# BlueSwordM/aom-av1-psy

Measured on AMD Instinct MI355X. Metric: SAD-candidates/s, higher is better.
Workload: dtype u8; 1 GPU; sad16x16_modeA_1080p_8bit; frame=1920x1080, bit_depth=8, block=16x16, mode=A: 1 sad16x16 @mv(0,0) + 1 sad16x16x4d (uniform in [-64,64]^2) per block, ring_frame_pairs_per_gpu=64, partition=uniform tile columns (tile_common.c:76-97), one per GPU; no data-path collective

## Files before the change

aom-av1-psy_amd/csrc/sad_sb.hip:

```cpp
#include <type_traits>

#include "common.h"
#include "variance_device.h"
#undef AOMHIP_FOR_BLOCK_SIZES

namespace aomhip {
namespace sb {

template <bool VAR> struct Ac;
template <> struct Ac<false> { uint32_t a = 0; };
template <> struct Ac<true> { uint32_t a = 0, rr = 0, xr = 0, ssum = 0, ss = 0; };
template <bool VAR> struct Res;
template <> struct Res<false> { uint32_t v; };
template <> struct Res<true> { uint32_t v, sse; };
template <typename T> __device__ __forceinline__ uint32_t dot_dword(uint32_t a, uint32_t b, uint32_t acc) {
  if constexpr (sizeof(T) == 1) return __builtin_amdgcn_udot4(a, b, acc, false);
  else return __builtin_amdgcn_udot2(__builtin_bit_cast(__attribute__((__vector_size__(2 * sizeof(unsigned short)))) unsigned short, a),
                                     __builtin_bit_cast(__attribute__((__vector_size__(2 * sizeof(unsigned short)))) unsigned short, b), acc, false);
}

struct __attribute__((packed, aligned(1))) U128 { uint32_t v[4]; };
struct __attribute__((packed, aligned(1))) U64 { uint32_t v[2]; };
struct __attribute__((packed, aligned(1))) U32 { uint32_t v[1]; };
template <int BYTES> struct UnitLoad;
template <> struct UnitLoad<16> { using type = U128; using aligned_type = uint4; };
template <> struct UnitLoad<8> { using type = U64; using aligned_type = uint2; };
template <> struct UnitLoad<4> { using type = U32; using aligned_type = uint32_t; };

template <typename T> __device__ __forceinline__ uint32_t sad_dword(uint32_t a, uint32_t b, uint32_t acc);
template <> __device__ __forceinline__ uint32_t sad_dword<uint8_t>(uint32_t a, uint32_t b, uint32_t acc) {
  return __builtin_amdgcn_sad_u8(a, b, acc);
}
template <> __device__ __forceinline__ uint32_t sad_dword<uint16_t>(uint32_t a, uint32_t b, uint32_t acc) {
  return __builtin_amdgcn_sad_u16(a, b, acc);
}

template <int TPC> __device__ __forceinline__ uint32_t group_sum(uint32_t v) {
  if constexpr (TPC >= 2) v += __builtin_amdgcn_update_dpp(0u, v, 0xB1, 0xf, 0xf, false);
  if constexpr (TPC >= 4) v += __builtin_amdgcn_update_dpp(0u, v, 0x4E, 0xf, 0xf, false);
  if constexpr (TPC >= 8) v += __builtin_amdgcn_update_dpp(0u, v, 0x141, 0xf, 0xf, false);
  if constexpr (TPC >= 16) v += __builtin_amdgcn_update_dpp(0u, v, 0x140, 0xf, 0xf, false);
  if constexpr (TPC >= 32) v += __shfl_xor(v, 16, 64);
  if constexpr (TPC >= 64) v += __shfl_xor(v, 32, 64);
  return v;
}

template <typename T, int W, int H, bool SKIP, int UPL> struct Geom {
  static constexpr int kRowBytes = W * (int)sizeof(T);
  static constexpr int kUnitBytes = kRowBytes < 16 ? kRowBytes : 16;
  static constexpr int kUnitElems = kUnitBytes / (int)sizeof(T);
  static constexpr int kUnitsPerRow = kRowBytes / kUnitBytes;
  static constexpr int kRows = SKIP ? H / 2 : H;
  static constexpr int kUnits = kUnitsPerRow * kRows;
  static constexpr int kTpcRaw = UPL > 0 ? (kUnits >= UPL ? kUnits / UPL : 1) : (kUnits < 16 ? kUnits : 16);
  static constexpr int kTpc = kTpcRaw > 64 ? 64 : kTpcRaw;
  static constexpr int kUnitsPerLane = kUnits / kTpc;
  static constexpr int kRowStep = SKIP ? 2 : 1;
};

template <int BYTES>
__device__ __forceinline__ typename UnitLoad<BYTES>::type lds_unit(const char *lds, unsigned byte_off) {
  const uint32_t *p = reinterpret_cast<const uint32_t *>(lds) + (byte_off >> 2);
  const unsigned sh = byte_off & 3;
  uint32_t d[BYTES / 4 + 1];
#pragma unroll
  for (int i = 0; i <= BYTES / 4; ++i) d[i] = p[i];
  typename UnitLoad<BYTES>::type out;
#pragma unroll
  for (int i = 0; i < BYTES / 4; ++i) out.v[i] = __builtin_amdgcn_alignbyte(d[i + 1], d[i], sh);
  return out;
}
template <int BYTES>
__device__ __forceinline__ typename UnitLoad<BYTES>::type lds_unit_aligned(const char *lds, unsigned byte_off) {
  using A = typename UnitLoad<BYTES>::aligned_type;
  const A t = *reinterpret_cast<const A *>(lds + byte_off);
  typename UnitLoad<BYTES>::type out;
  memcpy(&out, &t, BYTES);
  return out;
}

struct StripArgs {
  int first_frame, n_frames;
  int sb_w, sb_h, range, cells_per_row, cell_rows;
  int xmin, xmax, ymin, ymax, row_end, border;
  int s_xmax, s_ymax, s_row_end, s_border;
  int cpr, pitch, R;
  int scpr, spitch;
  unsigned magic_cpr, magic_scpr, magic_R;
  int ring_off, src_off[2], gdesc_off[2], cdesc_off[2], misc_off, seg_off;
  int gcap, ccap;
  int shift;
  int dbg;
};

__device__ __forceinline__ int uni(int v) { return __builtin_amdgcn_readfirstlane(v); }

#ifndef AOMHIP_SB_DBG_KNOBS
#define AOMHIP_SB_DBG_KNOBS 0
#endif
#ifdef AOMHIP_SB_PROF
__device__ unsigned long long g_sb_prof[32];
#define SB_T(v) const long long v = (long long)__builtin_readcyclecounter()
#define SB_ACC(i, t1, t0) prof_acc[i] += (unsigned long long)((t1) - (t0))
#define SB_DECL unsigned long long prof_acc[8] = { 0, 0, 0, 0, 0, 0, 0, 0 }, prof_wait = 0
#define SB_WAIT(t1, t0) prof_wait += (unsigned long long)((t1) - (t0))
#define SB_FLUSH if (tid == 0 || tid == kThreads) { for (int i_ = 0; i_ < 8; ++i_) atomicAdd(&g_sb_prof[(tid ? 8 : 0) + i_], prof_acc[i_]); } \
  if (lane == 0) atomicAdd(&g_sb_prof[16 + wave], prof_wait);
#else
#define SB_DECL
#define SB_FLUSH
#define SB_T(v)
#define SB_ACC(i, t1, t0)
#define SB_WAIT(t1, t0)
#endif

constexpr int kMirrorMax = 15;
__host__ __device__ constexpr int mirror_rows(int h) { return h - 1 <= kMirrorMax ? h - 1 : 0; }

template <int EVAL, int UPL_, int LOADERS, int RING_N, int SRC_N, int G_N, int C_N> struct Cfg {
  static constexpr int kThreads = EVAL, kUPL = UPL_, kLoaders = LOADERS, kRingN = RING_N, kSrcN = SRC_N, kGN = G_N, kCN = C_N;
  static constexpr int kLT = 64 * LOADERS / 2;
  static constexpr int kAll = EVAL + 64 * LOADERS;
};
using CfgWide = Cfg<512, 2, 8, 6, 4, 2, 1>;
using CfgDeep = Cfg<768, 1, 4, 9, 6, 4, 2>;
template <typename T, int W, int H, bool SKIP, typename C, bool VAR = false>
__global__ __launch_bounds__(C::kAll) void sad_strip_kernel(PlaneView<T> src, PlaneView<T> ref, StripArgs a,
                                                                  const aomhip_sad_x4d_cand *__restrict__ groups,
                                                                  const int32_t *__restrict__ group_off, int n_groups,
                                                                  int64_t group_frame_stride, uint32_t *__restrict__ out4,
                                                                  const aomhip_sad_cand *__restrict__ cands,
                                                                  const int32_t *__restrict__ cand_off, int n_cands,
                                                                  int64_t cand_frame_stride, uint32_t *__restrict__ out1,
                                                                  uint32_t *__restrict__ out4b = nullptr, uint32_t *__restrict__ out1b = nullptr) {
  static_assert(!VAR || (!SKIP && W * H <= 256), "the variance form: whole blocks of at most 256 pixels (32-bit sums)");
  constexpr int kThreads = C::kThreads, UPL = C::kUPL, kRingN = C::kRingN, kSrcN = C::kSrcN, kGN = C::kGN,
                kCN = C::kCN, kLT = C::kLT;
  using G = Geom<T, W, H, SKIP, UPL>;
  using L = typename UnitLoad<G::kUnitBytes>::type;
  extern __shared__ __attribute__((aligned(16))) char lds[];
  constexpr int kES = (int)sizeof(T);
  constexpr int kEpc = 16 / kES;
  constexpr int kPerWg = kThreads / G::kTpc;
  constexpr int kWaves = kThreads / 64;
  constexpr int kAll = C::kAll;
  constexpr int kGenUnroll = G::kUnitsPerLane <= 4 ? G::kUnitsPerLane : 4;
  constexpr int kMirror = mirror_rows(H);
  const int tid = (int)threadIdx.x;
#if AOMHIP_SB_DBG_KNOBS
  const int dbg = a.dbg;
#else
  constexpr int dbg = 0;
#endif
  const int lane = tid & 63;
  const int wave = uni(tid >> 6);
  const bool is_loader = wave >= kWaves;
  const int grp = uni((tid - kThreads) / kLT);
  const int lt = tid - kThreads - grp * kLT;
  const int lane_in_cand = tid % G::kTpc;
  const int slot = tid / G::kTpc;

  int *misc = reinterpret_cast<int *>(lds + a.misc_off);
  uint8_t *active = reinterpret_cast<uint8_t *>(misc + 72);
  for (int i = tid; i < 72; i += kAll) misc[i] = 0;
  __syncthreads();
  {
    const int n_buckets = a.cells_per_row * a.cell_rows;
    for (int b = tid; b < n_buckets; b += kAll) {
      int n = 0;
      if (groups) n += group_off[b + 1] - group_off[b];
      if (cands) n += cand_off[b + 1] - cand_off[b];
      if (n > 0) {
        const int cx = b % a.cells_per_row;
        atomicOr(reinterpret_cast<unsigned *>(&misc[8 + (cx >> 5)]), 1u << (cx & 31));
      }
    }
    __syncthreads();
    if (tid < 64) {
      int count = 0;
      for (int base = 0; base < a.cells_per_row; base += 64) {
        const int cx = base + tid;
        const bool f = cx < a.cells_per_row && ((misc[8 + (cx >> 5)] >> (cx & 31)) & 1);
        const unsigned long long m = __ballot(f);
        if (f) active[count + __popcll(m & ((1ull << tid) - 1))] = (uint8_t)cx;
        count += __popcll(m);
      }
      if (tid == 0) misc[0] = count;
    }
    __syncthreads();
  }
  const int n_active = uni(misc[0]);
  if (n_active == 0) return;
  const int src_off0 = a.src_off[0], src_off1 = a.src_off[1], gdesc_off0 = a.gdesc_off[0], gdesc_off1 = a.gdesc_off[1];
  const int cdesc_off0 = a.cdesc_off[0], cdesc_off1 = a.cdesc_off[1];
  auto src_off_of = [&](int buf) { return buf ? src_off1 : src_off0; };
  auto gdesc_off_of = [&](int buf) { return buf ? gdesc_off1 : gdesc_off0; };
  auto cdesc_off_of = [&](int buf) { return buf ? cdesc_off1 : cdesc_off0; };

  auto run = [&](auto role) {
    constexpr bool kLoader = decltype(role)::value;
    constexpr bool kTab = G::kUnitsPerLane <= 4;
    constexpr int kTabN = kTab ? G::kUnitsPerLane : 1;
    int unit_row_t[kTabN], unit_colb_t[kTabN];
    unsigned unit_roff_t[kTabN], unit_soff_t[kTabN];
    if constexpr (kTab) {
  #pragma unroll
      for (int k = 0; k < G::kUnitsPerLane; ++k) {
        const int u = lane_in_cand + k * G::kTpc;
        unit_row_t[k] = (u / G::kUnitsPerRow) * G::kRowStep;
        unit_colb_t[k] = (u % G::kUnitsPerRow) * G::kUnitBytes;
        unit_roff_t[k] = (unsigned)(unit_row_t[k] * a.pitch + unit_colb_t[k]);
        unit_soff_t[k] = (unsigned)(unit_row_t[k] * a.spitch + unit_colb_t[k]);
      }
    }
    auto unit_row = [&](int k) -> int {
      if constexpr (kTab) return unit_row_t[k]; else return ((lane_in_cand + k * G::kTpc) / G::kUnitsPerRow) * G::kRowStep;
    };
    auto unit_colb = [&](int k) -> int {
      if constexpr (kTab) return unit_colb_t[k]; else return ((lane_in_cand + k * G::kTpc) % G::kUnitsPerRow) * G::kUnitBytes;
    };
    auto unit_roff = [&](int k) -> unsigned {
      if constexpr (kTab) return unit_roff_t[k]; else return (unsigned)(unit_row(k) * a.pitch + unit_colb(k));
    };
    auto unit_soff = [&](int k) -> unsigned {
      if constexpr (kTab) return unit_soff_t[k]; else return (unsigned)(unit_row(k) * a.spitch + unit_colb(k));
    };

    const bool affine = a.n_frames >= 8;
    const int xcd = affine ? (int)(blockIdx.x & 7) : 0;
    const int wg_j = affine ? (int)(blockIdx.x >> 3) : (int)blockIdx.x;
    const int wg_n = affine ? (int)(gridDim.x >> 3) : (int)gridDim.x;
    const int frames_here = affine ? (a.n_frames - xcd + 7) >> 3 : a.n_frames;
    const int n_items = frames_here * n_active;

    SB_DECL;
    for (int item = wg_j; item < n_items; item += wg_n) {
      const int fi = item / n_active;
      const int f_rel = affine ? xcd + 8 * fi : fi;
      const int cx = uni((int)active[item - fi * n_active]);
      const int cell_x0 = cx * a.sb_w;
      const int wx0 = max(((cell_x0 - a.range + a.border) & ~(kEpc - 1)) - a.border, a.xmin);
      const int colmax = min(a.cpr - 1, (a.row_end - wx0) / kEpc - 1);
      const int wx1 = min(wx0 + (colmax + 1) * kEpc, a.xmax);
      const int sx0 = ((cell_x0 + a.s_border) & ~(kEpc - 1)) - a.s_border;
      const int scolmax = min(a.scpr - 1, (a.s_row_end - sx0) / kEpc - 1);
      const int sx1 = min(sx0 + (scolmax + 1) * kEpc, a.s_xmax);
      const char *ref_frame = reinterpret_cast<const char *>(ref.origin + (int64_t)(a.first_frame + f_rel) * ref.frame_stride);
      const char *src_frame = reinterpret_cast<const char *>(src.origin + (int64_t)(a.first_frame + f_rel) * src.frame_stride);
      const int gpitch = ref.stride * kES, sgpitch = src.stride * kES;
      const aomhip_sad_x4d_cand *glist = groups ? groups + (int64_t)f_rel * group_frame_stride : nullptr;
      const aomhip_sad_cand *clist = cands ? cands + (int64_t)f_rel * cand_frame_stride : nullptr;

      struct Batch { int ya, yb, sy0, ns, g0, ng, c0, nc, buf; unsigned first; };
      typedef uint32_t V4 __attribute__((ext_vector_type(4)));
      struct Stage { V4 ring[kRingN]; V4 srcv[kSrcN]; uint32_t g[kGN]; uint32_t c[kCN]; };
      const uint32_t *gwords = groups ? reinterpret_cast<const uint32_t *>(glist) : reinterpret_cast<const uint32_t *>(ref_frame);
      const uint32_t *cwords = cands ? reinterpret_cast<const uint32_t *>(clist) : reinterpret_cast<const uint32_t *>(ref_frame);
      const int gwords_n = groups ? n_groups * 5 : 1, cwords_n = cands ? n_cands * 2 : 1;
      auto request_gen = [&](const Batch &b, Stage &st, int me, int n) {
        const int total_r = (b.yb - b.ya) * a.cpr, total_s = b.ns * a.scpr;
        const char *rb = ref_frame + (int64_t)b.ya * gpitch + (int64_t)wx0 * kES;
        const char *sb_ = src_frame + (int64_t)b.sy0 * sgpitch + (int64_t)sx0 * kES;
  #pragma unroll
        for (int i = 0; i < kRingN; ++i) {
          const unsigned q = (unsigned)max(min(me + i * n, total_r - 1), 0);
          const unsigned row = __umulhi(q, a.magic_cpr), col = q - row * (unsigned)a.cpr;
          st.ring[i] = *reinterpret_cast<const V4 *>(rb + (row * (unsigned)gpitch + (unsigned)min((int)col, colmax) * 16u));
        }
  #pragma unroll
        for (int i = 0; i < kSrcN; ++i) {
          const unsigned q = (unsigned)max(min(me + i * n, total_s - 1), 0);
          const unsigned row = __umulhi(q, a.magic_scpr), col = q - row * (unsigned)a.scpr;
          st.srcv[i] = *reinterpret_cast<const V4 *>(sb_ + (row * (unsigned)sgpitch + (unsigned)min((int)col, scolmax) * 16u));
        }
  #pragma unroll
        for (int i = 0; i < kGN; ++i) st.g[i] = gwords[(unsigned)max(min(b.g0 * 5 + min(me + i * n, b.ng * 5 - 1), gwords_n - 1), 0)];
  #pragma unroll
        for (int i = 0; i < kCN; ++i) st.c[i] = cwords[(unsigned)max(min(b.c0 * 2 + min(me + i * n, b.nc * 2 - 1), cwords_n - 1), 0)];
      };
      auto commit_gen = [&](const Batch &b, const Stage &st, int me, int n) {
        const int total_r = (b.yb - b.ya) * a.cpr, total_s = b.ns * a.scpr;
        const unsigned s_first = (unsigned)((b.ya - a.ymin) % a.R);
  #pragma unroll
        for (int i = 0; i < kRingN; ++i) {
          const unsigned q = (unsigned)(me + i * n);
          if ((int)q < total_r) {
            const unsigned row = __umulhi(q, a.magic_cpr), col = q - row * (unsigned)a.cpr;
            unsigned sl = s_first + row;
            sl = min(sl, sl - (unsigned)a.R);
            const V4 v = st.ring[i];
            *reinterpret_cast<V4 *>(lds + a.ring_off + sl * a.pitch + col * 16) = v;
            if (kMirror > 0 && sl < (unsigned)kMirror)
              *reinterpret_cast<V4 *>(lds + a.ring_off + (sl + a.R) * a.pitch + col * 16) = v;
          }
        }
  #pragma unroll
        for (int i = 0; i < kSrcN; ++i) {
          const unsigned q = (unsigned)(me + i * n);
          if ((int)q < total_s) {
            const unsigned row = __umulhi(q, a.magic_scpr), col = q - row * (unsigned)a.scpr;
            *reinterpret_cast<V4 *>(lds + src_off_of(b.buf) + row * a.spitch + col * 16) = st.srcv[i];
          }
        }
  #pragma unroll
        for (int i = 0; i < kGN; ++i)
          if (me + i * n < b.ng * 5) *reinterpret_cast<uint32_t *>(lds + gdesc_off_of(b.buf) + (me + i * n) * 4) = st.g[i];
  #pragma unroll
        for (int i = 0; i < kCN; ++i)
          if (me + i * n < b.nc * 2) *reinterpret_cast<uint32_t *>(lds + cdesc_off_of(b.buf) + (me + i * n) * 4) = st.c[i];
      };
      auto win_y0 = [&](int cy) { return max(cy * a.sb_h - a.range, a.ymin); };
      auto win_y1 = [&](int cy) { return min(cy * a.sb_h + a.sb_h + a.range, a.ymax); };
      struct Seg { int g0, g1, c0, c1; };
      const int4 *segs = reinterpret_cast<const int4 *>(lds + a.seg_off);
      int4 *wins = reinterpret_cast<int4 *>(lds + a.seg_off) + a.cell_rows, *bats = wins + a.cell_rows;
      auto seg_of = [&](int cy) {
        const int4 v = segs[cy];
        Seg s;
        s.g0 = uni(v.x); s.g1 = uni(v.y); s.c0 = uni(v.z); s.c1 = uni(v.w);
        return s;
      };
      struct Win { int wy0, s0; unsigned wh_ok, sy0, sh_ok; };
      const unsigned ww_ok = (unsigned)(wx1 - wx0 - W), sw_ok = (unsigned)(sx1 - sx0 - W);
      const bool strip_ok = wx1 - wx0 >= W && sx1 - sx0 >= W;
      auto global_unit = [&](const char *frame, int pitch_b, int x, int y, int k) {
        return *reinterpret_cast<const L *>(frame + (int64_t)(y + unit_row(k)) * pitch_b + (int64_t)x * kES + unit_colb(k));
      };
      using AcT = Ac<VAR>;
      using ResT = Res<VAR>;
      auto add_ref = [&](uint32_t sd, uint32_t rd, AcT &acc) {
        if constexpr (VAR) {
          acc.a = sad_dword<T>(rd, 0u, acc.a);
          acc.rr = dot_dword<T>(rd, rd, acc.rr);
          acc.xr = dot_dword<T>(sd, rd, acc.xr);
        } else {
          acc.a = sad_dword<T>(sd, rd, acc.a);
        }
      };
      auto add_src = [&](uint32_t sd, uint32_t &ssum, uint32_t &ss) {
        ssum = sad_dword<T>(sd, 0u, ssum);
        ss = dot_dword<T>(sd, sd, ss);
      };
      auto sad_unit = [&](const L &s, const L &r, AcT acc) {
  #pragma unroll
        for (int i = 0; i < G::kUnitBytes / 4; ++i) {
          add_ref(s.v[i], r.v[i], acc);
          if constexpr (VAR) add_src(s.v[i], acc.ssum, acc.ss);
        }
        return acc;
      };
      auto reduce = [&](const AcT &acc) {
        ResT r;
        if constexpr (VAR) {
          const uint32_t dsum = group_sum<G::kTpc>(acc.ssum - acc.a);
          const uint32_t q = group_sum<G::kTpc>(acc.ss + acc.rr - 2u * acc.xr);
          finish<(sizeof(T) > 1), ilog2v(W * H)>((int64_t)(int32_t)dsum, (uint64_t)q, 8 + a.shift, &r.v, &r.sse);
        } else {
          r.v = ((SKIP ? 2u * group_sum<G::kTpc>(acc.a) : group_sum<G::kTpc>(acc.a)) >> a.shift);
        }
        return r;
      };
// ... 213 lines not shown
                  const L sv = lds_unit_aligned<G::kUnitBytes>(sbuf, soff + unit_soff(k));
                  if constexpr (kKeepSrc) gsrc[k] = sv;
  #pragma unroll
                  for (int j = 0; j < 4; ++j) acc[j] = sad_unit(sv, ring_unit(base[j], slot0[j], k), acc[j]);
                }
              } else {
  #pragma unroll kGenUnroll
                for (int k = 0; k < G::kUnitsPerLane; ++k) {
                  const L sv = lds_unit<G::kUnitBytes>(sbuf, soff + unit_soff(k));
                  if constexpr (kKeepSrc) gsrc[k] = sv;
  #pragma unroll
                  for (int j = 0; j < 4; ++j) acc[j] = sad_unit(sv, ring_unit(base[j], slot0[j], k), acc[j]);
                }
              }
              gsrc_ok = kKeepSrc;
            } else {
  #pragma unroll 1
              for (int j = 0; j < 4; ++j) {
                int jrx = rx[j], jry = ry[j];
                if constexpr (kCoop) {
                  jrx = (int)quad_bcast((unsigned)rx[0], j);
                  jry = (int)quad_bcast((unsigned)ry[0], j);
                }
                const AcT v = generic_ref(gsx, gsy, jrx, jry);
#pragma unroll
                for (int q = 0; q < 4; ++q) {
                  acc[q].a = j == q ? v.a : acc[q].a;
                  if constexpr (VAR) {
                    acc[q].rr = j == q ? v.rr : acc[q].rr; acc[q].xr = j == q ? v.xr : acc[q].xr;
                    acc[q].ssum = j == q ? v.ssum : acc[q].ssum; acc[q].ss = j == q ? v.ss : acc[q].ss;
                  }
                }
              }
            }
            const ResT r0 = reduce(acc[0]), r1 = reduce(acc[1]), r2 = reduce(acc[2]), r3 = reduce(acc[3]);
            if (lane_in_cand == 0) store_group((int64_t)f_rel * n_groups + g0 + i, r0, r1, r2, r3);
          }
          if (has_c) {
            const uint32_t d0 = cd[i * 2], d1 = cd[i * 2 + 1];
            const int sx = (int16_t)d0, sy = (int16_t)(d0 >> 16), rx = (int16_t)d1, ry = (int16_t)(d1 >> 16);
            AcT acc;
            unsigned soff, base;
            int slot0;
            bool in = src_pos(w, sx, sy, soff);
            in = ring_pos(w, rx, ry, base, slot0) && in;
            if (in) {
              const bool reuse = gsrc_ok && sx == gsx && sy == gsy;
              if (__all(reuse)) {
                if constexpr (kKeepSrc) {
  #pragma unroll
                  for (int k = 0; k < G::kUnitsPerLane; ++k) acc = sad_unit(gsrc[k], ring_unit(base, slot0, k), acc);
                }
              } else {
  #pragma unroll kGenUnroll
                for (int k = 0; k < G::kUnitsPerLane; ++k)
                  acc = sad_unit(lds_unit<G::kUnitBytes>(sbuf, soff + unit_soff(k)), ring_unit(base, slot0, k), acc);
              }
            } else {
              acc = generic_ref(sx, sy, rx, ry);
            }
            const ResT rc = reduce(acc);
            if (lane_in_cand == 0) store_cand((int64_t)f_rel * n_cands + c0 + i, rc);
          }
        }
      };

      auto batch_of = [&](int cy) {
        const bool real = cy < a.cell_rows;
        const int cyc = real ? cy : a.cell_rows - 1;
        const Seg sg = seg_of(cyc);
        const int4 bv = bats[cyc];
        Batch b;
        b.ya = uni(bv.x);
        b.yb = real ? b.ya + uni(bv.y) : b.ya;
        b.sy0 = cyc * a.sb_h; b.ns = real ? uni(bv.z) : 0;
        b.first = (unsigned)uni(bv.w);
        b.g0 = sg.g0; b.ng = real ? min(sg.g1 - sg.g0, a.gcap) : 0;
        b.c0 = sg.c0; b.nc = real ? min(sg.c1 - sg.c0, a.ccap) : 0;
        b.buf = cy & 1;
        if ((dbg & 2) && cy > 0) { b.yb = b.ya; b.ns = 0; }
        if (dbg & 8192) { b.ng = 0; b.nc = 0; }
        return b;
      };
      int crowded = 0;
      for (int cy = tid; cy < a.cell_rows; cy += kAll) {
        const int b = cy * a.cells_per_row + cx;
        const int4 sg = make_int4(groups ? group_off[b] : 0, groups ? group_off[b + 1] : 0, cands ? cand_off[b] : 0, cands ? cand_off[b + 1] : 0);
        reinterpret_cast<int4 *>(lds + a.seg_off)[cy] = sg;
        crowded |= (sg.y - sg.x > a.gcap) | (sg.w - sg.z > a.ccap);
        const int wy0 = win_y0(cy), wy1 = win_y1(cy);
        const int sh = min(cy * a.sb_h + a.sb_h, a.s_ymax) - cy * a.sb_h;
        const bool ok = strip_ok && wy1 - wy0 >= H && sh >= H;
        const unsigned wh_ok = strip_ok && wy1 - wy0 >= H ? (unsigned)(wy1 - wy0 - H) : 0u;
        wins[cy] = make_int4(wy0, (wy0 - a.ymin) % a.R, (int)wh_ok, (int)(((unsigned)(sh - H) & 0x7fffffffu) | (ok ? 0x80000000u : 0u)));
        const int ya = cy > 0 ? win_y1(cy - 1) : win_y0(0);
        bats[cy] = make_int4(ya, wy1 - ya, sh, ((ya - a.ymin) % a.R) * a.pitch);
      }
      if (lane == 0) misc[16 + wave] = __ballot(crowded != 0) != 0 ? 1 : 0;
      __syncthreads();
      bool any_crowded;
      {
        const int4 *f = reinterpret_cast<const int4 *>(misc + 16);
        const int4 f0 = f[0], f1 = f[1], f2 = f[2], f3 = f[3];
        any_crowded = uni((f0.x | f0.y | f0.z | f0.w | f1.x | f1.y | f1.z | f1.w | f2.x | f2.y | f2.z | f2.w | f3.x | f3.y | f3.z | f3.w)) != 0;
      }
      SB_T(p0);
      {
        Stage st0;
        const int rows_per_pass = (kRingN * kAll) / a.cpr;
        const Batch b = batch_of(0);
        for (int ya = win_y0(0); ya < win_y1(0); ya += rows_per_pass) {
          Batch p = b;
          p.ya = ya; p.yb = min(ya + rows_per_pass, win_y1(0));
          if (ya != win_y0(0)) { p.ns = 0; p.ng = 0; p.nc = 0; }
          int me = tid;
          asm volatile("" : "+v"(me));
          request_gen(p, st0, me, kAll);
          commit_gen(p, st0, me, kAll);
        }
      }
      unsigned r_goff[kRingN], r_loff[kRingN], s_goff[kSrcN], s_loff[kSrcN];
      int lt_s = lt;
      asm volatile("" : "+v"(lt_s));
#pragma unroll
      for (int i = 0; i < kRingN; ++i) {
        const unsigned q = (unsigned)(lt_s + i * kLT), row = __umulhi(q, a.magic_cpr), col = q - row * (unsigned)a.cpr;
        r_goff[i] = row * (unsigned)gpitch + (unsigned)min((int)col, colmax) * 16u;
        r_loff[i] = row * (unsigned)a.pitch + col * 16u;
      }
  #pragma unroll
      for (int i = 0; i < kSrcN; ++i) {
        const unsigned q = (unsigned)(lt_s + i * kLT), row = __umulhi(q, a.magic_scpr), col = q - row * (unsigned)a.scpr;
        s_goff[i] = row * (unsigned)sgpitch + (unsigned)min((int)col, scolmax) * 16u;
        s_loff[i] = row * (unsigned)a.spitch + col * 16u;
      }
      const unsigned ring_bytes = (unsigned)(a.R * a.pitch);
      auto request = [&](const Batch &b, Stage &st) {
        const char *rb = ref_frame + (int64_t)min(b.ya, a.ymax - 1) * gpitch + (int64_t)wx0 * kES;
        const char *sb_ = src_frame + (int64_t)min(b.sy0, a.s_ymax - 1) * sgpitch + (int64_t)sx0 * kES;
        const unsigned rlim = (unsigned)((b.yb - b.ya) * gpitch), slim = (unsigned)(b.ns * sgpitch);
  #pragma unroll
        for (int i = 0; i < kRingN; ++i) st.ring[i] = *reinterpret_cast<const V4 *>(rb + (r_goff[i] < rlim ? r_goff[i] : 0u));
  #pragma unroll
        for (int i = 0; i < kSrcN; ++i) st.srcv[i] = *reinterpret_cast<const V4 *>(sb_ + (s_goff[i] < slim ? s_goff[i] : 0u));
  #pragma unroll
        for (int i = 0; i < kGN; ++i) st.g[i] = gwords[(unsigned)max(min(b.g0 * 5 + min(lt + i * kLT, b.ng * 5 - 1), gwords_n - 1), 0)];
  #pragma unroll
        for (int i = 0; i < kCN; ++i) st.c[i] = cwords[(unsigned)max(min(b.c0 * 2 + min(lt + i * kLT, b.nc * 2 - 1), cwords_n - 1), 0)];
      };
      auto commit = [&](const Batch &b, const Stage &st) {
        const unsigned rlim = (unsigned)((b.yb - b.ya) * gpitch), slim = (unsigned)(b.ns * sgpitch);
        const unsigned first = b.first;
        const bool mirrored = kMirror > 0 && (first < (unsigned)(kMirror * a.pitch) || first + (unsigned)(b.yb - b.ya) * (unsigned)a.pitch > ring_bytes);
        if (mirrored) {
  #pragma unroll
          for (int i = 0; i < kRingN; ++i)
            if (r_goff[i] < rlim) {
              unsigned t = first + r_loff[i];
              t = min(t, t - ring_bytes);
              const V4 v = st.ring[i];
              *reinterpret_cast<V4 *>(lds + a.ring_off + t) = v;
              if (t < (unsigned)(kMirror * a.pitch)) *reinterpret_cast<V4 *>(lds + a.ring_off + t + ring_bytes) = v;
            }
        } else {
  #pragma unroll
          for (int i = 0; i < kRingN; ++i)
            if (r_goff[i] < rlim) *reinterpret_cast<V4 *>(lds + a.ring_off + first + r_loff[i]) = st.ring[i];
        }
  #pragma unroll
        for (int i = 0; i < kSrcN; ++i)
          if (s_goff[i] < slim)
            *reinterpret_cast<V4 *>(lds + src_off_of(b.buf) + s_loff[i]) = st.srcv[i];
  #pragma unroll
        for (int i = 0; i < kGN; ++i)
          if (lt + i * kLT < b.ng * 5) *reinterpret_cast<uint32_t *>(lds + gdesc_off_of(b.buf) + (lt + i * kLT) * 4) = st.g[i];
  #pragma unroll
        for (int i = 0; i < kCN; ++i)
          if (lt + i * kLT < b.nc * 2) *reinterpret_cast<uint32_t *>(lds + cdesc_off_of(b.buf) + (lt + i * kLT) * 4) = st.c[i];
      };
      const int steps = (dbg & 256) ? 0 : (a.cell_rows + 1) & ~1;
      if constexpr (kLoader) {
        Stage st;
        auto overflow = [&](int cy, bool mine) {
          if (cy >= a.cell_rows) return;
          const Seg cur = seg_of(cy);
          int g = cur.g0 + min(cur.g1 - cur.g0, a.gcap), c = cur.c0 + min(cur.c1 - cur.c0, a.ccap);
          while (g < cur.g1 || c < cur.c1) {
            Batch o;
            o.ya = o.yb = win_y0(0); o.sy0 = 0; o.ns = 0; o.buf = cy & 1;
            o.g0 = g; o.ng = min(cur.g1 - g, a.gcap); o.c0 = c; o.nc = min(cur.c1 - c, a.ccap);
            __syncthreads();
            if (mine) {
              int me = lt;
              asm volatile("" : "+v"(me));
              Stage so;
              request_gen(o, so, me, kLT);
              commit_gen(o, so, me, kLT);
            }
            __syncthreads();
            g += o.ng; c += o.nc;
          }
        };
        Batch held = batch_of(0);
        auto active = [&](int cy) {
          if (dbg & 64) { __syncthreads(); return; }
          SB_T(l0);
          const Batch bc = held;
          SB_T(l1);
#ifdef AOMHIP_SB_PROF
          asm volatile("s_waitcnt vmcnt(0)" ::: "memory");
          SB_T(l1w);
          SB_ACC(7, l1w, l1);
#endif
          commit(bc, st);
          SB_T(l2);
          if (any_crowded) overflow(cy, true);
          SB_T(l3);
          __syncthreads();
          SB_T(l5);
          SB_ACC(0, l1, l0); SB_ACC(1, l2, l1); SB_ACC(2, l3, l2); SB_ACC(4, l5, l3); SB_ACC(5, 1, 0); SB_WAIT(l5, l3);
        };
        auto passive = [&](int cy) {
          if (dbg & 64) { __syncthreads(); return; }
          SB_T(q0);
          held = batch_of(cy + 2);
          request(held, st);
          SB_T(q1);
          if (any_crowded) overflow(cy, false);
          __syncthreads();
          SB_T(q2);
          SB_ACC(3, q1, q0); SB_ACC(6, q2, q1); SB_WAIT(q2, q1);
        };
        if (grp == 0) {
          held = batch_of(1);
          request(held, st);
          __syncthreads();
          for (int cy = 0; cy < steps; cy += 2) {
            active(cy);
            passive(cy + 1);
          }
        } else {
          __syncthreads();
          for (int cy = 0; cy < steps; cy += 2) {
            passive(cy);
            active(cy + 1);
          }
        }
      } else {
        __syncthreads();
        SB_T(p1);
        SB_ACC(5, p1, p0); SB_ACC(6, 1, 0);
        for (int cy = 0; cy < steps; ++cy) {
          if (cy >= a.cell_rows) {
            __syncthreads();
            break;
          }
          if (dbg & (64 | 2048)) { __syncthreads(); continue; }
          const int buf = cy & 1;
          SB_T(t1);
          const Seg cur = seg_of(cy);
          const int4 wv = wins[cy];
          Win w;
          w.wy0 = uni(wv.x);
          w.s0 = uni(wv.y);
          w.wh_ok = (unsigned)uni(wv.z);
          w.sy0 = (unsigned)(cy * a.sb_h);
          w.sh_ok = (unsigned)uni(wv.w) & 0x7fffffffu;
          const bool step_ok = (unsigned)uni(wv.w) >> 31;
          int g = cur.g0, c = cur.c0;
          bool first = true;
          SB_T(t1b);
          SB_ACC(0, t1b, t1);
          do {
            const int ng = min(cur.g1 - g, a.gcap), nc = min(cur.c1 - c, a.ccap);
            if (!first) {
              __syncthreads();
              __syncthreads();
            }
            if (!(dbg & 1)) {
              if (step_ok) {
                eval(w, buf, g, ng, c, nc);
              } else {
                for (int gi = slot; gi < ng; gi += kPerWg) {
                  const uint32_t *e = reinterpret_cast<const uint32_t *>(glist + g + gi);
                  const uint32_t e0 = e[0], e1 = e[1], e2 = e[2], e3 = e[3], e4 = e[4];
                  const int sx = (int16_t)e0, sy = (int16_t)(e0 >> 16);
                  const ResT r0 = reduce(generic_ref(sx, sy, (int16_t)e1, (int16_t)e3));
                  const ResT r1 = reduce(generic_ref(sx, sy, (int16_t)(e1 >> 16), (int16_t)(e3 >> 16)));
                  const ResT r2 = reduce(generic_ref(sx, sy, (int16_t)e2, (int16_t)e4));
                  const ResT r3 = reduce(generic_ref(sx, sy, (int16_t)(e2 >> 16), (int16_t)(e4 >> 16)));
                  if (lane_in_cand == 0) store_group((int64_t)f_rel * n_groups + g + gi, r0, r1, r2, r3);
                }
                for (int ci = slot; ci < nc; ci += kPerWg) {
                  const uint32_t *e = reinterpret_cast<const uint32_t *>(clist + c + ci);
                  const uint32_t e0 = e[0], e1 = e[1];
                  const ResT v = reduce(generic_ref((int16_t)e0, (int16_t)(e0 >> 16), (int16_t)e1, (int16_t)(e1 >> 16)));
                  if (lane_in_cand == 0) store_cand((int64_t)f_rel * n_cands + c + ci, v);
                }
              }
            }
            g += ng; c += nc;
            first = false;
          } while (g < cur.g1 || c < cur.c1);
          SB_T(t2);
          __syncthreads();
          SB_T(t4);
          SB_ACC(1, t2, t1); SB_ACC(3, t4, t2); SB_ACC(4, 1, 0); SB_WAIT(t4, t2);
        }
      }
    }
    SB_FLUSH;
  };
  if (wave >= kWaves / 2 && wave < kWaves) __builtin_amdgcn_s_setprio(1);
  if (is_loader) run(std::true_type{}); else run(std::false_type{});
}

struct SbLaunch {
  hipStream_t stream;
  int grid, threads, upl;
  bool deep;
  size_t lds_bytes;
  StripArgs a;
  const aomhip_sad_x4d_cand *groups;
  const int32_t *group_off;
  int n_groups;
  int64_t gfs;
  uint32_t *out4;
  const aomhip_sad_cand *cands;
  const int32_t *cand_off;
  int n_cands;
  int64_t cfs;
  uint32_t *out1;
  uint32_t *out4b, *out1b;
  bool var;
};

template <typename T, int W, int H, bool SKIP, typename C, bool VAR = false>
static int launch_nt(const SbLaunch &l, const PlaneView<T> &s, const PlaneView<T> &r) {
  auto k = sad_strip_kernel<T, W, H, SKIP, C, VAR>;
  static thread_local size_t granted = 0;
  if (l.lds_bytes > granted) {
    AOMHIP_TRY(hipFuncSetAttribute(reinterpret_cast<const void *>(k), hipFuncAttributeMaxDynamicSharedMemorySize,
                                   (int)l.lds_bytes));
    granted = l.lds_bytes;
  }
  hipLaunchKernelGGL(k, dim3((unsigned)l.grid), dim3(C::kAll), l.lds_bytes, l.stream, s, r, l.a,
                     l.groups, l.group_off, l.n_groups, l.gfs, l.out4, l.cands, l.cand_off, l.n_cands, l.cfs, l.out1, l.out4b, l.out1b);
  AOMHIP_LAUNCH_CHECK();
  return AOMHIP_OK;
}

constexpr bool deep_size(int es, int w, int h) { return es == 1 && w == 16 && h == 16; }
inline bool use_deep(int es, int w, int h, bool skip) {
  if (!deep_size(es, w, h) || skip) return false;
  const char *e = getenv("AOMHIP_SB_CFG");
  return e && e[0] == 'd';
}
template <typename T, int W, int H, bool SKIP>
static int launch(const SbLaunch &l, const PlaneView<T> &s, const PlaneView<T> &r) {
  if constexpr (deep_size((int)sizeof(T), W, H) && !SKIP) {
    if (l.deep) return launch_nt<T, W, H, SKIP, CfgDeep>(l, s, r);
  }
  return launch_nt<T, W, H, SKIP, CfgWide>(l, s, r);
}

#ifdef AOMHIP_SB_ONLY_16
#define AOMHIP_FOR_BLOCK_SIZES(X) X(16, 16)
#else
#define AOMHIP_FOR_BLOCK_SIZES(X)                                                                                \
  X(4, 4) X(4, 8) X(8, 4) X(8, 8) X(8, 16) X(16, 8) X(16, 16) X(16, 32) X(32, 16) X(32, 32) X(32, 64) X(64, 32) \
  X(64, 64) X(64, 128) X(128, 64) X(128, 128) X(4, 16) X(16, 4) X(8, 32) X(32, 8) X(16, 64) X(64, 16)
#endif

#ifdef AOMHIP_SB_ONLY_16
#define AOMHIP_FOR_VAR_BLOCK_SIZES(X) X(16, 16)
#else
#define AOMHIP_FOR_VAR_BLOCK_SIZES(X) X(4, 4) X(4, 8) X(8, 4) X(8, 8) X(8, 16) X(16, 8) X(16, 16) X(4, 16) X(16, 4) X(8, 32) X(32, 8)
#endif

template <typename T>
static int dispatch(const SbLaunch &l, bool skip, const PlaneView<T> &s, const PlaneView<T> &r, int bw, int bh) {
  if (l.var) {
#define X(W, H) \
  if (bw == W && bh == H) return launch_nt<T, W, H, false, CfgWide, true>(l, s, r);
    AOMHIP_FOR_VAR_BLOCK_SIZES(X)
#undef X
    set_error("aomhip_variance_sb_batch: blocks of at most 256 pixels (%dx%d): use aomhip_variance_batch", bw, bh);
    return AOMHIP_ERR_INVALID;
  }
#define X(W, H) \
  if (bw == W && bh == H) return skip ? launch<T, W, H, (H >= 2)>(l, s, r) : launch<T, W, H, false>(l, s, r);
  AOMHIP_FOR_BLOCK_SIZES(X)
#undef X
  set_error("unsupported block size %dx%d", bw, bh);
  return AOMHIP_ERR_INVALID;
}

static unsigned magic_of(int d) { return (unsigned)((0x100000000ull + (unsigned)d - 1) / (unsigned)d); }

}
}

using namespace aomhip;

#ifdef AOMHIP_SB_PROF
extern "C" int aomhip_debug_sb_prof(unsigned long long out[32], int reset) {
  if (hipMemcpyFromSymbol(out, HIP_SYMBOL(sb::g_sb_prof), 256) != hipSuccess) return AOMHIP_ERR_HIP;
  if (reset) { unsigned long long z[32] = {0}; if (hipMemcpyToSymbol(HIP_SYMBOL(sb::g_sb_prof), z, 256) != hipSuccess) return AOMHIP_ERR_HIP; }
  return AOMHIP_OK;
}
#endif

static int sb_batch(aomhip_ctx *ctx, const aomhip_planes *src, const aomhip_planes *ref, int first_frame,
                    int n_frames, int bw, int bh, int flags, int sb_w, int sb_h, int range,
                    int n_buckets, const aomhip_sad_x4d_cand *d_groups,
                    const int32_t *d_group_bucket_offsets, int n_groups, int64_t group_frame_stride,
                    uint32_t *d_out_groups, const aomhip_sad_cand *d_cands,
                    const int32_t *d_cand_bucket_offsets, int n_cands, int64_t cand_frame_stride,
                    uint32_t *d_out_cands, bool var, uint32_t *d_out_groups_b, uint32_t *d_out_cands_b) {
  if (!ctx || !src || !ref || !src->base || !ref->base) {
    set_error("null argument");
    return AOMHIP_ERR_INVALID;
  }
  if ((d_groups && (!d_group_bucket_offsets || !d_out_groups || (var && !d_out_groups_b))) ||
      (d_cands && (!d_cand_bucket_offsets || !d_out_cands || (var && !d_out_cands_b))) || (!d_groups && !d_cands) || (var && flags != 0)) {
    set_error("a list needs its bucket offsets and its output array; at least one list is required");
    return AOMHIP_ERR_INVALID;
  }
  if (!valid_block(bw, bh)) {
    set_error("unsupported block size %dx%d", bw, bh);
    return AOMHIP_ERR_INVALID;
  }
  if (src->bit_depth != ref->bit_depth && !(src->bit_depth > 8 && ref->bit_depth > 8)) {
    set_error("src/ref element types differ");
    return AOMHIP_ERR_INVALID;
  }
  if (n_groups < 0 || n_cands < 0 || n_frames < 0 || first_frame < 0 || first_frame + n_frames > src->n_frames ||
      first_frame + n_frames > ref->n_frames) {
    set_error("frame range out of bounds");
    return AOMHIP_ERR_INVALID;
  }
  if (sb_w < 1 || sb_h < 1 || range < 0 || n_buckets < 0) {
    set_error("bad bucket geometry");
    return AOMHIP_ERR_INVALID;
  }
  const int cells_per_row = (src->width + sb_w - 1) / sb_w;
  const int cell_rows = (src->height + sb_h - 1) / sb_h;
  if (n_buckets != cells_per_row * cell_rows) {
    set_error("n_buckets %d != %d x %d cells of %dx%d over a %dx%d plane", n_buckets, cells_per_row, cell_rows, sb_w, sb_h,
              src->width, src->height);
    return AOMHIP_ERR_INVALID;
  }
  if (cells_per_row > 256) {
    set_error("at most 256 cells per row (%d of width %d)", cells_per_row, sb_w);
    return AOMHIP_ERR_INVALID;
  }
  if (n_buckets == 0 || n_frames == 0) return AOMHIP_OK;
  const int es = ref->bit_depth > 8 ? 2 : 1, epc = 16 / es;
  sb::SbLaunch l;
  sb::StripArgs &a = l.a;
  memset(&a, 0, sizeof(a));
  const bool aligned = (sb_w % epc) == 0 && (range % epc) == 0 && (ref->border % epc) == 0;
  a.cpr = ((sb_w + 2 * range) * es + 15) / 16 + (aligned ? 0 : 1);
  a.pitch = (a.cpr | 1) * 16;
  a.R = 2 * sb_h + 2 * range;
  a.scpr = (sb_w * es + 15) / 16 + (((sb_w % epc) == 0 && (src->border % epc) == 0) ? 0 : 1);
  a.spitch = ((a.scpr & 3) == 0 ? a.scpr + 1 : a.scpr) * 16;
  l.deep = sb::use_deep(es, bw, bh, (flags & AOMHIP_SAD_SKIP_ROWS) != 0);
  const int ring_chunks = l.deep ? sb::CfgDeep::kRingN * sb::CfgDeep::kLT : sb::CfgWide::kRingN * sb::CfgWide::kLT;
  const int src_chunks = l.deep ? sb::CfgDeep::kSrcN * sb::CfgDeep::kLT : sb::CfgWide::kSrcN * sb::CfgWide::kLT;
  const int g_words = l.deep ? sb::CfgDeep::kGN * sb::CfgDeep::kLT : sb::CfgWide::kGN * sb::CfgWide::kLT;
  const int c_words = l.deep ? sb::CfgDeep::kCN * sb::CfgDeep::kLT : sb::CfgWide::kCN * sb::CfgWide::kLT;
  if (sb_h * a.cpr > ring_chunks || sb_h * a.scpr > src_chunks) {
    set_error("a step of %d rows x (%d + %d) bytes exceeds what the loader wavefronts keep in flight (%d + %d KB): use a lower cell",
              sb_h, a.cpr * 16, a.scpr * 16, ring_chunks / 64, src_chunks / 64);
    return AOMHIP_ERR_INVALID;
  }
  const size_t ring_bytes = (size_t)(a.R + sb::mirror_rows(bh)) * a.pitch, cell_bytes = (size_t)sb_h * a.spitch;
  const size_t kLds = 160 * 1024, misc_bytes = 72 * 4 + 256 + (size_t)cell_rows * 48 + 16;
  if (ring_bytes + 2 * cell_bytes + misc_bytes + 4 * 256 > kLds) {
    set_error("LDS ring of %d rows x %d bytes + two %d x %d source cells (%zu bytes) exceed the 160 KB LDS of a CU: "
              "use a lower cell (sb_h) or a narrower one", a.R, a.pitch, sb_w, sb_h, ring_bytes + 2 * cell_bytes);
    return AOMHIP_ERR_INVALID;
  }
  {
    size_t per_buf = (kLds - ring_bytes - 2 * cell_bytes - misc_bytes) / 2;
    if (per_buf > 16 * 1024) per_buf = 16 * 1024;
    int cap = (int)((per_buf - 32) / 28);
    if (cap > g_words / 5) cap = g_words / 5;
    if (cap > c_words / 2) cap = c_words / 2;
    if (const char *e = getenv("AOMHIP_SB_DESC_CAP")) cap = atoi(e) < cap && atoi(e) > 0 ? atoi(e) : cap;
    a.gcap = a.ccap = cap;
    size_t off = 0;
    a.ring_off = 0; off += ring_bytes;
    for (int i = 0; i < 2; ++i) { a.src_off[i] = (int)off; off += cell_bytes; }
    for (int i = 0; i < 2; ++i) {
      a.gdesc_off[i] = (int)off; off += ((size_t)cap * 20 + 15) & ~(size_t)15;
      a.cdesc_off[i] = (int)off; off += ((size_t)cap * 8 + 15) & ~(size_t)15;
    }
    a.misc_off = (int)off; a.seg_off = (int)((off + 72 * 4 + 256 + 15) & ~(size_t)15); off += misc_bytes;
    l.lds_bytes = (off + 15) & ~(size_t)15;
  }
  a.magic_cpr = sb::magic_of(a.cpr); a.magic_scpr = sb::magic_of(a.scpr); a.magic_R = sb::magic_of(a.R);
  a.first_frame = first_frame; a.n_frames = n_frames;
  a.sb_w = sb_w; a.sb_h = sb_h; a.range = range; a.cells_per_row = cells_per_row; a.cell_rows = cell_rows;
  a.xmin = -ref->border; a.xmax = ref->width + ref->border; a.ymin = -ref->border; a.ymax = ref->height + ref->border;
  a.row_end = ref->stride - ref->border; a.border = ref->border;
  a.s_xmax = src->width + src->border; a.s_ymax = src->height + src->border; a.s_row_end = src->stride - src->border;
  a.s_border = src->border;
  a.shift = src->bit_depth == 10 ? 2 : src->bit_depth == 12 ? 4 : 0;
  if (const char *e = getenv("AOMHIP_SB_DBG")) a.dbg = atoi(e);
  l.stream = ctx->stream;
  {
    static thread_local int cus = 0;
    if (!cus) {
      hipDeviceProp_t prop;
      AOMHIP_TRY(hipGetDeviceProperties(&prop, ctx->device));
      cus = prop.multiProcessorCount > 0 ? prop.multiProcessorCount : 256;
    }
    const int per_cu = (int)(kLds / l.lds_bytes) < 1 ? 1 : (int)(kLds / l.lds_bytes);
    l.threads = per_cu >= 2 ? 512 : 1024;
    int grid = cus * (per_cu > 2 ? 2 : per_cu);
    if (const char *e = getenv("AOMHIP_SB_THREADS")) l.threads = atoi(e);
    if (const char *e = getenv("AOMHIP_SB_GRID")) grid = atoi(e);
    grid &= ~7;
    if (grid < 8) grid = 8;
    const int items = n_frames * cells_per_row;
    if (n_frames < 8 && grid > items) grid = items;
    l.grid = grid;
  }
  l.groups = n_groups > 0 ? d_groups : nullptr; l.group_off = d_group_bucket_offsets; l.n_groups = n_groups; l.gfs = group_frame_stride;
  l.out4 = d_out_groups;
  l.cands = n_cands > 0 ? d_cands : nullptr; l.cand_off = d_cand_bucket_offsets; l.n_cands = n_cands; l.cfs = cand_frame_stride;
  l.out1 = d_out_cands;
  l.var = var; l.out4b = d_out_groups_b; l.out1b = d_out_cands_b;
  const bool skip = (flags & AOMHIP_SAD_SKIP_ROWS) != 0;
  if (src->bit_depth == 8) return sb::dispatch<uint8_t>(l, skip, view_of<uint8_t>(*src), view_of<uint8_t>(*ref), bw, bh);
  return sb::dispatch<uint16_t>(l, skip, view_of<uint16_t>(*src), view_of<uint16_t>(*ref), bw, bh);
}

extern "C" int aomhip_sad_sb_batch(aomhip_ctx *ctx, const aomhip_planes *src, const aomhip_planes *ref, int first_frame,
                                   int n_frames, int bw, int bh, int flags, int sb_w, int sb_h, int range,
                                   int n_buckets, const aomhip_sad_x4d_cand *d_groups,
                                   const int32_t *d_group_bucket_offsets, int n_groups, int64_t group_frame_stride,
                                   uint32_t *d_out_groups, const aomhip_sad_cand *d_cands,
                                   const int32_t *d_cand_bucket_offsets, int n_cands, int64_t cand_frame_stride,
                                   uint32_t *d_out_cands) {
  return sb_batch(ctx, src, ref, first_frame, n_frames, bw, bh, flags, sb_w, sb_h, range, n_buckets, d_groups, d_group_bucket_offsets, n_groups,
                  group_frame_stride, d_out_groups, d_cands, d_cand_bucket_offsets, n_cands, cand_frame_stride, d_out_cands, false, nullptr, nullptr);
}

extern "C" int aomhip_variance_sb_batch(aomhip_ctx *ctx, const aomhip_planes *src, const aomhip_planes *ref, int first_frame, int n_frames, int bw,
                                        int bh, int sb_w, int sb_h, int range, int n_buckets, const aomhip_sad_x4d_cand *d_groups,
                                        const int32_t *d_group_bucket_offsets, int n_groups, int64_t group_frame_stride, uint32_t *d_var_groups,
                                        uint32_t *d_sse_groups, const aomhip_sad_cand *d_cands, const int32_t *d_cand_bucket_offsets, int n_cands,
                                        int64_t cand_frame_stride, uint32_t *d_var_cands, uint32_t *d_sse_cands) {
  return sb_batch(ctx, src, ref, first_frame, n_frames, bw, bh, 0, sb_w, sb_h, range, n_buckets, d_groups, d_group_bucket_offsets, n_groups,
                  group_frame_stride, d_var_groups, d_cands, d_cand_bucket_offsets, n_cands, cand_frame_stride, d_var_cands, true, d_sse_groups,
                  d_sse_cands);
}
```

Before: 33.62 billion candidates/s.

## Cache bucket offsets in LDS and overlap prologue loads with setup

The kernel now copies the group and candidate bucket offsets into LDS during the initial scan, when the extra LDS fits without lowering occupancy, so later per-row segment lookups read LDS instead of global memory. The first window prefetch for cell row 0 is issued earlier, before the segment table and loader offset computations, so its global latency overlaps that setup. The prologue also drops an extra __syncthreads that came after the first batch request. Profiling hooks are extended with prologue timers. The costs are more LDS use and a reordered prologue whose synchronisation must stay correct.

```diff
diff --git a/aom-av1-psy_amd/csrc/sad_sb.hip b/aom-av1-psy_amd/csrc/sad_sb.hip
--- a/aom-av1-psy_amd/csrc/sad_sb.hip
+++ b/aom-av1-psy_amd/csrc/sad_sb.hip
@@ -88,6 +88,7 @@
   int scpr, spitch;
   unsigned magic_cpr, magic_scpr, magic_R;
   int ring_off, src_off[2], gdesc_off[2], cdesc_off[2], misc_off, seg_off;
+  int boff_off;
   int gcap, ccap;
   int shift;
   int dbg;
@@ -99,12 +100,15 @@
 #define AOMHIP_SB_DBG_KNOBS 0
 #endif
 #ifdef AOMHIP_SB_PROF
-__device__ unsigned long long g_sb_prof[32];
+__device__ unsigned long long g_sb_prof[40];
 #define SB_T(v) const long long v = (long long)__builtin_readcyclecounter()
 #define SB_ACC(i, t1, t0) prof_acc[i] += (unsigned long long)((t1) - (t0))
-#define SB_DECL unsigned long long prof_acc[8] = { 0, 0, 0, 0, 0, 0, 0, 0 }, prof_wait = 0
+#define SB_DECL unsigned long long prof_acc[8] = { 0, 0, 0, 0, 0, 0, 0, 0 }, prof_pro[8] = { 0, 0, 0, 0, 0, 0, 0, 0 }, prof_wait = 0
+#define SB_PRO(i, t1, t0) prof_pro[i] += (unsigned long long)((t1) - (t0))
+#define SB_DRAIN asm volatile("s_waitcnt vmcnt(0)" ::: "memory")
 #define SB_WAIT(t1, t0) prof_wait += (unsigned long long)((t1) - (t0))
-#define SB_FLUSH if (tid == 0 || tid == kThreads) { for (int i_ = 0; i_ < 8; ++i_) atomicAdd(&g_sb_prof[(tid ? 8 : 0) + i_], prof_acc[i_]); } \
+#define SB_FLUSH if (tid == 0 || tid == kThreads) { for (int i_ = 0; i_ < 8; ++i_) atomicAdd(&g_sb_prof[(tid ? 8 : 0) + i_], prof_acc[i_]); \
+    for (int i_ = (tid ? 6 : 0); i_ < (tid ? 8 : 6); ++i_) atomicAdd(&g_sb_prof[32 + i_], prof_pro[i_]); } \
   if (lane == 0) atomicAdd(&g_sb_prof[16 + wave], prof_wait);
 #else
 #define SB_DECL
@@ -112,6 +116,8 @@
 #define SB_T(v)
 #define SB_ACC(i, t1, t0)
 #define SB_WAIT(t1, t0)
+#define SB_PRO(i, t1, t0)
+#define SB_DRAIN
 #endif
 
 constexpr int kMirrorMax = 15;
@@ -162,14 +168,20 @@
 
   int *misc = reinterpret_cast<int *>(lds + a.misc_off);
   uint8_t *active = reinterpret_cast<uint8_t *>(misc + 72);
+  SB_T(sc0);
   for (int i = tid; i < 72; i += kAll) misc[i] = 0;
   __syncthreads();
   {
     const int n_buckets = a.cells_per_row * a.cell_rows;
+    int *boff = reinterpret_cast<int *>(lds + max(a.boff_off, 0));
     for (int b = tid; b < n_buckets; b += kAll) {
-      int n = 0;
-      if (groups) n += group_off[b + 1] - group_off[b];
-      if (cands) n += cand_off[b + 1] - cand_off[b];
+      const int g0 = groups ? group_off[b] : 0, g1 = groups ? group_off[b + 1] : 0;
+      const int c0 = cands ? cand_off[b] : 0, c1 = cands ? cand_off[b + 1] : 0;
+      if (a.boff_off >= 0) {
+        boff[b] = g0; boff[n_buckets + 1 + b] = c0;
+        if (b == n_buckets - 1) { boff[b + 1] = g1; boff[n_buckets + 2 + b] = c1; }
+      }
+      const int n = (g1 - g0) + (c1 - c0);
       if (n > 0) {
         const int cx = b % a.cells_per_row;
         atomicOr(reinterpret_cast<unsigned *>(&misc[8 + (cx >> 5)]), 1u << (cx & 31));
@@ -190,6 +202,7 @@
     __syncthreads();
   }
   const int n_active = uni(misc[0]);
+  SB_T(sc1);
   if (n_active == 0) return;
   const int src_off0 = a.src_off[0], src_off1 = a.src_off[1], gdesc_off0 = a.gdesc_off[0], gdesc_off1 = a.gdesc_off[1];
   const int cdesc_off0 = a.cdesc_off[0], cdesc_off1 = a.cdesc_off[1];
@@ -234,6 +247,7 @@
     const int n_items = frames_here * n_active;
 
     SB_DECL;
+    SB_PRO(0, sc1, sc0);
     for (int item = wg_j; item < n_items; item += wg_n) {
       const int fi = item / n_active;
       const int f_rel = affine ? xcd + 8 * fi : fi;
@@ -257,7 +271,7 @@
       const uint32_t *gwords = groups ? reinterpret_cast<const uint32_t *>(glist) : reinterpret_cast<const uint32_t *>(ref_frame);
       const uint32_t *cwords = cands ? reinterpret_cast<const uint32_t *>(clist) : reinterpret_cast<const uint32_t *>(ref_frame);
       const int gwords_n = groups ? n_groups * 5 : 1, cwords_n = cands ? n_cands * 2 : 1;
-      auto request_gen = [&](const Batch &b, Stage &st, int me, int n) {
+      auto request_gen_px = [&](const Batch &b, Stage &st, int me, int n) {
         const int total_r = (b.yb - b.ya) * a.cpr, total_s = b.ns * a.scpr;
         const char *rb = ref_frame + (int64_t)b.ya * gpitch + (int64_t)wx0 * kES;
         const char *sb_ = src_frame + (int64_t)b.sy0 * sgpitch + (int64_t)sx0 * kES;
@@ -273,10 +287,16 @@
           const unsigned row = __umulhi(q, a.magic_scpr), col = q - row * (unsigned)a.scpr;
           st.srcv[i] = *reinterpret_cast<const V4 *>(sb_ + (row * (unsigned)sgpitch + (unsigned)min((int)col, scolmax) * 16u));
         }
+      };
+      auto request_gen_ls = [&](const Batch &b, Stage &st, int me, int n) {
   #pragma unroll
         for (int i = 0; i < kGN; ++i) st.g[i] = gwords[(unsigned)max(min(b.g0 * 5 + min(me + i * n, b.ng * 5 - 1), gwords_n - 1), 0)];
   #pragma unroll
         for (int i = 0; i < kCN; ++i) st.c[i] = cwords[(unsigned)max(min(b.c0 * 2 + min(me + i * n, b.nc * 2 - 1), cwords_n - 1), 0)];
+      };
+      auto request_gen = [&](const Batch &b, Stage &st, int me, int n) {
+        request_gen_px(b, st, me, n);
+        request_gen_ls(b, st, me, n);
       };
       auto commit_gen = [&](const Batch &b, const Stage &st, int me, int n) {
         const int total_r = (b.yb - b.ya) * a.cpr, total_s = b.ns * a.scpr;
@@ -656,10 +676,36 @@
         if (dbg & 8192) { b.ng = 0; b.nc = 0; }
         return b;
       };
+      SB_T(r0);
+      Stage st0;
+      const int rows_per_pass = (kRingN * kAll) / a.cpr, wy0_0 = win_y0(0), wy1_0 = win_y1(0);
+      const int nb1 = a.cells_per_row * a.cell_rows + 1;
+      const int *boff = reinterpret_cast<const int *>(lds + max(a.boff_off, 0));
+      const bool boff_lds = a.boff_off >= 0;
+      int me0 = tid;
+      asm volatile("" : "+v"(me0));
+      Batch pb;
+      pb.ya = wy0_0; pb.yb = min(wy0_0 + rows_per_pass, wy1_0); pb.sy0 = 0; pb.ns = min(a.sb_h, a.s_ymax); pb.first = 0u; pb.buf = 0;
+      request_gen_px(pb, st0, me0, kAll);
+      {
+        int g0, g1, c0, c1;
+        if (boff_lds) {
+          g0 = boff[cx]; g1 = boff[cx + 1]; c0 = boff[nb1 + cx]; c1 = boff[nb1 + cx + 1];
+        } else {
+          g0 = groups ? group_off[cx] : 0; g1 = groups ? group_off[cx + 1] : 0; c0 = cands ? cand_off[cx] : 0; c1 = cands ? cand_off[cx + 1] : 0;
+        }
+        pb.g0 = uni(g0); pb.ng = min(uni(g1) - pb.g0, a.gcap);
+        pb.c0 = uni(c0); pb.nc = min(uni(c1) - pb.c0, a.ccap);
+        if (dbg & 8192) { pb.ng = 0; pb.nc = 0; }
+      }
+      request_gen_ls(pb, st0, me0, kAll);
+      SB_T(a1);
       int crowded = 0;
       for (int cy = tid; cy < a.cell_rows; cy += kAll) {
         const int b = cy * a.cells_per_row + cx;
-        const int4 sg = make_int4(groups ? group_off[b] : 0, groups ? group_off[b + 1] : 0, cands ? cand_off[b] : 0, cands ? cand_off[b + 1] : 0);
+        int4 sg;
+        if (boff_lds) sg = make_int4(boff[b], boff[b + 1], boff[nb1 + b], boff[nb1 + b + 1]);
+        else sg = make_int4(groups ? group_off[b] : 0, groups ? group_off[b + 1] : 0, cands ? cand_off[b] : 0, cands ? cand_off[b + 1] : 0);
         reinterpret_cast<int4 *>(lds + a.seg_off)[cy] = sg;
         crowded |= (sg.y - sg.x > a.gcap) | (sg.w - sg.z > a.ccap);
         const int wy0 = win_y0(cy), wy1 = win_y1(cy);
@@ -671,42 +717,43 @@
         bats[cy] = make_int4(ya, wy1 - ya, sh, ((ya - a.ymin) % a.R) * a.pitch);
       }
       if (lane == 0) misc[16 + wave] = __ballot(crowded != 0) != 0 ? 1 : 0;
+      SB_T(a1r);
+      unsigned r_goff[kRingN], r_loff[kRingN], s_goff[kSrcN], s_loff[kSrcN];
+      int lt_s = lt;
+      asm volatile("" : "+v"(lt_s));
+#pragma unroll
+      for (int i = 0; i < kRingN; ++i) {
+        const unsigned q = (unsigned)(lt_s + i * kLT), row = __umulhi(q, a.magic_cpr), col = q - row * (unsigned)a.cpr;
+        r_goff[i] = row * (unsigned)gpitch + (unsigned)min((int)col, colmax) * 16u;
+        r_loff[i] = row * (unsigned)a.pitch + col * 16u;
+      }
+  #pragma unroll
+      for (int i = 0; i < kSrcN; ++i) {
+        const unsigned q = (unsigned)(lt_s + i * kLT), row = __umulhi(q, a.magic_scpr), col = q - row * (unsigned)a.scpr;
+        s_goff[i] = row * (unsigned)sgpitch + (unsigned)min((int)col, scolmax) * 16u;
+        s_loff[i] = row * (unsigned)a.spitch + col * 16u;
+      }
+      SB_T(a1t);
+      SB_DRAIN;
+      SB_T(a2);
+      commit_gen(pb, st0, me0, kAll);
+      for (int ya = pb.yb; ya < wy1_0; ya += rows_per_pass) {
+        Batch p = pb;
+        p.ya = ya; p.yb = min(ya + rows_per_pass, wy1_0);
+        p.ns = 0; p.ng = 0; p.nc = 0;
+        request_gen(p, st0, me0, kAll);
+        commit_gen(p, st0, me0, kAll);
+      }
+      SB_T(p2);
       __syncthreads();
+      SB_T(p1);
+      SB_PRO(2, a1, r0); SB_PRO(1, a1r, a1); SB_PRO(3, a2, a1t); SB_PRO(4, p2, a2); SB_PRO(5, p1, p2);
+      if (kLoader) { SB_PRO(6, a1t, a1r); SB_PRO(7, p1, p2); }
       bool any_crowded;
       {
         const int4 *f = reinterpret_cast<const int4 *>(misc + 16);
         const int4 f0 = f[0], f1 = f[1], f2 = f[2], f3 = f[3];
         any_crowded = uni((f0.x | f0.y | f0.z | f0.w | f1.x | f1.y | f1.z | f1.w | f2.x | f2.y | f2.z | f2.w | f3.x | f3.y | f3.z | f3.w)) != 0;
-      }
-      SB_T(p0);
-      {
-        Stage st0;
-        const int rows_per_pass = (kRingN * kAll) / a.cpr;
-        const Batch b = batch_of(0);
-        for (int ya = win_y0(0); ya < win_y1(0); ya += rows_per_pass) {
-          Batch p = b;
-          p.ya = ya; p.yb = min(ya + rows_per_pass, win_y1(0));
-          if (ya != win_y0(0)) { p.ns = 0; p.ng = 0; p.nc = 0; }
-          int me = tid;
-          asm volatile("" : "+v"(me));
-          request_gen(p, st0, me, kAll);
-          commit_gen(p, st0, me, kAll);
-        }
-      }
-      unsigned r_goff[kRingN], r_loff[kRingN], s_goff[kSrcN], s_loff[kSrcN];
-      int lt_s = lt;
-      asm volatile("" : "+v"(lt_s));
-#pragma unroll
-      for (int i = 0; i < kRingN; ++i) {
-        const unsigned q = (unsigned)(lt_s + i * kLT), row = __umulhi(q, a.magic_cpr), col = q - row * (unsigned)a.cpr;
-        r_goff[i] = row * (unsigned)gpitch + (unsigned)min((int)col, colmax) * 16u;
-        r_loff[i] = row * (unsigned)a.pitch + col * 16u;
-      }
-  #pragma unroll
-      for (int i = 0; i < kSrcN; ++i) {
-        const unsigned q = (unsigned)(lt_s + i * kLT), row = __umulhi(q, a.magic_scpr), col = q - row * (unsigned)a.scpr;
-        s_goff[i] = row * (unsigned)sgpitch + (unsigned)min((int)col, scolmax) * 16u;
-        s_loff[i] = row * (unsigned)a.spitch + col * 16u;
       }
       const unsigned ring_bytes = (unsigned)(a.R * a.pitch);
       auto request = [&](const Batch &b, Stage &st) {
@@ -808,22 +855,18 @@
         if (grp == 0) {
           held = batch_of(1);
           request(held, st);
-          __syncthreads();
           for (int cy = 0; cy < steps; cy += 2) {
             active(cy);
             passive(cy + 1);
           }
         } else {
-          __syncthreads();
           for (int cy = 0; cy < steps; cy += 2) {
             passive(cy);
             active(cy + 1);
           }
         }
       } else {
-        __syncthreads();
-        SB_T(p1);
-        SB_ACC(5, p1, p0); SB_ACC(6, 1, 0);
+        SB_ACC(5, p1, r0); SB_ACC(6, 1, 0);
         for (int cy = 0; cy < steps; ++cy) {
           if (cy >= a.cell_rows) {
             __syncthreads();
@@ -978,9 +1021,9 @@
 using namespace aomhip;
 
 #ifdef AOMHIP_SB_PROF
-extern "C" int aomhip_debug_sb_prof(unsigned long long out[32], int reset) {
-  if (hipMemcpyFromSymbol(out, HIP_SYMBOL(sb::g_sb_prof), 256) != hipSuccess) return AOMHIP_ERR_HIP;
-  if (reset) { unsigned long long z[32] = {0}; if (hipMemcpyToSymbol(HIP_SYMBOL(sb::g_sb_prof), z, 256) != hipSuccess) return AOMHIP_ERR_HIP; }
+extern "C" int aomhip_debug_sb_prof(unsigned long long out[40], int reset) {
+  if (hipMemcpyFromSymbol(out, HIP_SYMBOL(sb::g_sb_prof), 320) != hipSuccess) return AOMHIP_ERR_HIP;
+  if (reset) { unsigned long long z[40] = {0}; if (hipMemcpyToSymbol(HIP_SYMBOL(sb::g_sb_prof), z, 320) != hipSuccess) return AOMHIP_ERR_HIP; }
   return AOMHIP_OK;
 }
 #endif
@@ -1073,7 +1116,12 @@
       a.cdesc_off[i] = (int)off; off += ((size_t)cap * 8 + 15) & ~(size_t)15;
     }
     a.misc_off = (int)off; a.seg_off = (int)((off + 72 * 4 + 256 + 15) & ~(size_t)15); off += misc_bytes;
-    l.lds_bytes = (off + 15) & ~(size_t)15;
+    off = (off + 15) & ~(size_t)15;
+    const size_t boff_bytes = ((size_t)2 * (n_buckets + 1) * 4 + 15) & ~(size_t)15;
+    const char *e = getenv("AOMHIP_SB_BOFF_LDS");
+    a.boff_off = -1;
+    if (off + boff_bytes <= kLds && kLds / (off + boff_bytes) == kLds / off && !(e && atoi(e) == 0)) { a.boff_off = (int)off; off += boff_bytes; }
+    l.lds_bytes = off;
   }
   a.magic_cpr = sb::magic_of(a.cpr); a.magic_scpr = sb::magic_of(a.scpr); a.magic_R = sb::magic_of(a.R);
   a.first_frame = first_frame; a.n_frames = n_frames;
```

Result: faster. 34.01 billion candidates/s (median of 6 runs) (+1.2%).
